# YannDubs/disentangling-vae

Hardware: NVIDIA H100
Metric: images/sec (higher is better)
Workload: dtype f32

## Files before the change

### disentangling-vae_b200/csrc/dv_conv_tc.cu

```cuda
#include "dv_common.cuh"
#include "dv_ptx.cuh"

namespace dv {
namespace tc {

using namespace ptx;

constexpr int kATile = 128 * 128;
constexpr int kBTap = 64 * 128;
constexpr int kBBytes = kTaps * kBTap;
constexpr int kConsumers = 8;
constexpr int kThreads = (kConsumers + 1) * 32;
constexpr int kSmemMax = 232448;

__device__ __forceinline__ void consumers_sync() { asm volatile("bar.sync 1, %0;" ::"n"(kConsumers * 32) : "memory"); }

__device__ __forceinline__ int b_lane_row(int lane) { return (lane >> 4) * 32 + (lane & 7); }
__device__ __forceinline__ int b_lane_col(int lane) { return (lane & 8) >> 1; }
__device__ __forceinline__ void load_b_tap(uint32_t tap_base, int nt, int ks, int b_row, int b_col, uint32_t (&bh)[2], uint32_t (&bl)[2]) {
  uint32_t r[4];
  ldsm_x4(tap_base + swz128(b_row + 8 * nt, 8 * ks + b_col), r);
  bh[0] = r[0]; bh[1] = r[1]; bl[0] = r[2]; bl[1] = r[3];
}

struct DownGeom {
  int B, H, W;
  int rows_per_tile;
  int num_tiles;
  long long total_px;
};
constexpr int kDownStages = 5;
struct DownBarriers {
  uint64_t raw_full[kDownStages], raw_empty[kDownStages];
  uint64_t b_full;
  float bias[32];
  float csum[kConsumers][32];
};
constexpr int kDownSmem = kBBytes + kDownStages * kATile + 1024 + 2048;
static_assert(sizeof(DownBarriers) <= 2048, "barrier block too large");
static_assert(kDownSmem <= kSmemMax, "smem");

__global__ void __launch_bounds__(kThreads, 1)
conv_down32_mma_kernel(const __grid_constant__ CUtensorMap tmap_a, const __grid_constant__ CUtensorMap tmap_b,
                       const float* __restrict__ bias, const float* __restrict__ mask, float* __restrict__ lo,
                       DownGeom g, int act, float* __restrict__ colsum_part,
                       const uint32_t* __restrict__ mask_bits, uint32_t* __restrict__ bits_out) {
  extern __shared__ uint8_t smem_raw[];
  uint8_t* smem = align1024(smem_raw);
  uint8_t* Bs = smem;
  uint8_t* Raw = smem + kBBytes;
  DownBarriers* bars = reinterpret_cast<DownBarriers*>(Raw + kDownStages * kATile);
  const int warp = threadIdx.x >> 5, lane = threadIdx.x & 31;
  if (threadIdx.x == 0) {
    for (int s = 0; s < kDownStages; ++s) { mbar_init(&bars->raw_full[s], 1); mbar_init(&bars->raw_empty[s], kConsumers); }
    mbar_init(&bars->b_full, 1);
    fence_mbar_init();
  }
  if (threadIdx.x < 32) bars->bias[threadIdx.x] = bias ? bias[threadIdx.x] : 0.f;
  __syncthreads();

  if (warp == kConsumers) {
    if (lane != 0) return;
    prefetch_tmap(&tmap_a); prefetch_tmap(&tmap_b);
    mbar_arrive_expect_tx(&bars->b_full, kBBytes);
    for (int tap = 0; tap < kTaps; ++tap) tma_load_2d(Bs + tap * kBTap, &tmap_b, &bars->b_full, 0, tap * 64);
    int stage = 0; uint32_t phase = 0;
    for (int tile = blockIdx.x; tile < g.num_tiles; tile += gridDim.x) {
      const int r0 = tile * g.rows_per_tile;
      const int b0 = r0 / g.H, i0 = r0 % g.H;
      if (tile + (int)gridDim.x < g.num_tiles) {
        const int rn = (tile + gridDim.x) * g.rows_per_tile;
        const int bn = rn / g.H, in_ = rn % g.H;
        for (int t4 = 0; t4 < 4; ++t4) tma_prefetch_4d(&tmap_a, 0, (t4 & 1), 2 * in_ + (t4 >> 1), bn);
      }
      for (int tap = 0; tap < kTaps; ++tap) {
        const int kh = tap >> 2, kw = tap & 3;
        mbar_wait(&bars->raw_empty[stage], phase ^ 1);
        mbar_arrive_expect_tx(&bars->raw_full[stage], kATile);
        tma_load_4d(Raw + stage * kATile, &tmap_a, &bars->raw_full[stage], 0, kw - 1, 2 * i0 - 1 + kh, b0);
        if (++stage == kDownStages) { stage = 0; phase ^= 1; }
      }
    }
    return;
  }

  const int gq = lane >> 2, t = lane & 3;
  const int b_row = b_lane_row(lane), b_col = b_lane_col(lane);
  const int r0 = warp * 16 + gq;
  const uint32_t bs = smem_u32(Bs), raw0 = smem_u32(Raw);
  float csum[4][2] = {};
  mbar_wait(&bars->b_full, 0);
  int stage = 0; uint32_t phase = 0;
  for (int tile = blockIdx.x; tile < g.num_tiles; tile += gridDim.x) {
    float tot[4][4] = {}, corr[4][4] = {};
    for (int tap = 0; tap < kTaps; ++tap) {
      mbar_wait(&bars->raw_full[stage], phase);
      const uint32_t a_base = raw0 + stage * kATile, b_base = bs + tap * kBTap;
      float mn[4][4] = {};
#pragma unroll
      for (int ks = 0; ks < 4; ++ks) {
        uint32_t a[4], ah[4], al[4];
        a[0] = lds32(a_base + swz128(r0, 8 * ks + t));
        a[1] = lds32(a_base + swz128(r0 + 8, 8 * ks + t));
        a[2] = lds32(a_base + swz128(r0, 8 * ks + t + 4));
        a[3] = lds32(a_base + swz128(r0 + 8, 8 * ks + t + 4));
#pragma unroll
        for (int e = 0; e < 4; ++e) split_tf32(a[e], ah[e], al[e]);
#pragma unroll
        for (int nt = 0; nt < 4; ++nt) {
          uint32_t bh[2], bl[2];
          load_b_tap(b_base, nt, ks, b_row, b_col, bh, bl);
          mma_3xtf32(mn[nt], corr[nt], ah, al, bh, bl);
        }
      }
      __syncwarp();
      if (lane == 0) mbar_arrive(&bars->raw_empty[stage]);
      if (++stage == kDownStages) { stage = 0; phase ^= 1; }
#pragma unroll
      for (int nt = 0; nt < 4; ++nt)
#pragma unroll
        for (int e = 0; e < 4; ++e) tot[nt][e] += mn[nt][e];
    }
#pragma unroll
    for (int h = 0; h < 2; ++h) {
      const long long p = (long long)tile * 128 + r0 + 8 * h;
      const bool valid = p < g.total_px;
      uint32_t mb = 0xffffffffu;
      if (mask_bits && valid) mb = __ldg(mask_bits + p);
      const float* mk = (mask && !mask_bits && valid) ? mask + p * 32 : nullptr;
      uint32_t ob = 0u;
#pragma unroll
      for (int nt = 0; nt < 4; ++nt) {
        const int c = nt * 8 + 2 * t;
        float v[2];
#pragma unroll
        for (int e = 0; e < 2; ++e) {
          float x = (tot[nt][2 * h + e] + corr[nt][2 * h + e]) + bars->bias[c + e];
          if (act == DV_ACT_RELU) x = fmaxf(x, 0.f);
          v[e] = ((mb >> (c + e)) & 1u) ? x : 0.f;
        }
        if (mk) {
          const float2 m2 = __ldg(reinterpret_cast<const float2*>(mk + c));
          v[0] = m2.x > 0.f ? v[0] : 0.f; v[1] = m2.y > 0.f ? v[1] : 0.f;
        }
        if (valid) *reinterpret_cast<float2*>(lo + p * 32 + c) = make_float2(v[0], v[1]);
        else v[0] = v[1] = 0.f;
        ob |= (v[0] > 0.f ? 1u : 0u) << c | (v[1] > 0.f ? 1u : 0u) << (c + 1);
        csum[nt][0] += v[0]; csum[nt][1] += v[1];
      }
      ob |= __shfl_xor_sync(0xffffffffu, ob, 1);
      ob |= __shfl_xor_sync(0xffffffffu, ob, 2);
      if (bits_out && valid && t == 0) bits_out[p] = ob;
    }
  }
  if (colsum_part) {
#pragma unroll
    for (int nt = 0; nt < 4; ++nt)
#pragma unroll
      for (int e = 0; e < 2; ++e) {
        float s = csum[nt][e];
        s += __shfl_xor_sync(0xffffffffu, s, 4);
        s += __shfl_xor_sync(0xffffffffu, s, 8);
        s += __shfl_xor_sync(0xffffffffu, s, 16);
        if (gq == 0) bars->csum[warp][nt * 8 + 2 * t + e] = s;
      }
    consumers_sync();
    if (warp == 0) {
      float s = 0.f;
      for (int w = 0; w < kConsumers; ++w) s += bars->csum[w][lane];
      colsum_part[blockIdx.x * 32 + lane] = s;
    }
  }
}

constexpr int kWtSlots = kConsumers;
struct WtBarriers {
  uint64_t raw_full[kWtSlots], raw_empty[kWtSlots];
  uint64_t l_full[2], l_empty[2];
  float lsum[kConsumers][32];
};
constexpr int kWtTotFloats = 2 * 32 * 32;
constexpr int kWtSmem = kWtSlots * kATile + 2 * kATile + 2048 + kConsumers * kWtTotFloats * 4 + 1024;
static_assert(sizeof(WtBarriers) <= 2048, "barrier block too large");
static_assert(kWtSmem <= kSmemMax, "smem");

struct WtGeom {
  int B, H, W, rows_per_tile, num_tiles, tiles_per_cta;
};

__global__ void __launch_bounds__(kThreads, 1)
conv_wgrad32_mma_kernel(const __grid_constant__ CUtensorMap tmap_hi, const __grid_constant__ CUtensorMap tmap_lo,
                        float* __restrict__ ws, WtGeom g) {
  extern __shared__ uint8_t smem_raw[];
  uint8_t* smem = align1024(smem_raw);
  uint8_t* Raw = smem;
  uint8_t* Ls = smem + kWtSlots * kATile;
  WtBarriers* bars = reinterpret_cast<WtBarriers*>(Ls + 2 * kATile);
  const int warp = threadIdx.x >> 5, lane = threadIdx.x & 31;
  float* tot = reinterpret_cast<float*>(Ls + 2 * kATile + 2048) + warp * kWtTotFloats + lane;
  const int t_begin = blockIdx.x * g.tiles_per_cta;
  const int t_end = min(g.num_tiles, t_begin + g.tiles_per_cta);

  if (threadIdx.x == 0) {
    for (int s = 0; s < kWtSlots; ++s) { mbar_init(&bars->raw_full[s], 1); mbar_init(&bars->raw_empty[s], 1); }
    for (int s = 0; s < 2; ++s) { mbar_init(&bars->l_full[s], 1); mbar_init(&bars->l_empty[s], kConsumers); }
    fence_mbar_init();
  }
  __syncthreads();

  if (warp == kConsumers) {
    if (lane != 0) return;
    prefetch_tmap(&tmap_hi); prefetch_tmap(&tmap_lo);
    uint32_t tseq = 0;
    for (int tile = t_begin; tile < t_end; ++tile, ++tseq) {
      const int r0 = tile * g.rows_per_tile;
      const int b0 = r0 / g.H, i0 = r0 % g.H;
      if (tile + 1 < t_end) {
        const int rn = (tile + 1) * g.rows_per_tile;
        const int bn = rn / g.H, in_ = rn % g.H;
        for (int t4 = 0; t4 < 4; ++t4) tma_prefetch_4d(&tmap_hi, 0, (t4 & 1), 2 * in_ + (t4 >> 1), bn);
        tma_prefetch_4d(&tmap_lo, 0, 0, in_, bn);
      }
      const int lb = tseq & 1;
      mbar_wait(&bars->l_empty[lb], ((tseq >> 1) & 1u) ^ 1u);
      mbar_arrive_expect_tx(&bars->l_full[lb], kATile);
      tma_load_4d(Ls + lb * kATile, &tmap_lo, &bars->l_full[lb], 0, 0, i0, b0);
      for (int tap = 0; tap < kTaps; ++tap) {
        const int kh = tap >> 2, kw = tap & 3, slot = tap & 7;
        const uint32_t use = tseq * 2 + (tap >> 3);
        mbar_wait(&bars->raw_empty[slot], (use & 1u) ^ 1u);
        mbar_arrive_expect_tx(&bars->raw_full[slot], kATile);
        tma_load_4d(Raw + slot * kATile, &tmap_hi, &bars->raw_full[slot], 0, kw - 1, 2 * i0 - 1 + kh, b0);
      }
    }
    return;
  }

  const int gq = lane >> 2, t = lane & 3;
  const uint32_t slot_base = smem_u32(Raw) + warp * kATile, l0 = smem_u32(Ls);
  for (int k = 0; k < 64; ++k) tot[k * 32] = 0.f;
  float lsum = 0.f;
  uint32_t tseq = 0;
  for (int tile = t_begin; tile < t_end; ++tile, ++tseq) {
    const int lb = tseq & 1;
    mbar_wait(&bars->l_full[lb], (tseq >> 1) & 1u);
    const uint32_t l_base = l0 + lb * kATile;
#pragma unroll 4
    for (int r = 0; r < 16; ++r) lsum += __uint_as_float(lds32(l_base + swz128(warp * 16 + r, lane)));
#pragma unroll 1
    for (int j = 0; j < 2; ++j) {
      const uint32_t use = tseq * 2 + j;
      mbar_wait(&bars->raw_full[warp], use & 1u);
      float mn[2][4][4] = {}, cr[2][4][4] = {};
#pragma unroll 1
      for (int ks = 0; ks < 16; ++ks) {
        const int px0 = 8 * ks + 2 * t, px1 = px0 + 1;
        uint32_t ah[2][4], al[2][4], bh[4][2], bl[4][2];
#pragma unroll
        for (int mt = 0; mt < 2; ++mt) {
          const int c = mt * 16 + gq;
          uint32_t a[4];
          a[0] = lds32(slot_base + swz128(px0, c));
          a[1] = lds32(slot_base + swz128(px0, c + 8));
          a[2] = lds32(slot_base + swz128(px1, c));
          a[3] = lds32(slot_base + swz128(px1, c + 8));
#pragma unroll
          for (int e = 0; e < 4; ++e) split_tf32(a[e], ah[mt][e], al[mt][e]);
        }
#pragma unroll
        for (int nt = 0; nt < 4; ++nt) {
          const int cl = nt * 8 + gq;
          split_tf32(lds32(l_base + swz128(px0, cl)), bh[nt][0], bl[nt][0]);
          split_tf32(lds32(l_base + swz128(px1, cl)), bh[nt][1], bl[nt][1]);
        }
#pragma unroll
        for (int mt = 0; mt < 2; ++mt)
#pragma unroll
          for (int nt = 0; nt < 4; ++nt) mma_3xtf32(mn[mt][nt], cr[mt][nt], ah[mt], al[mt], bh[nt], bl[nt]);
      }
      __syncwarp();
      if (lane == 0) mbar_arrive(&bars->raw_empty[warp]);
#pragma unroll
      for (int mt = 0; mt < 2; ++mt)
#pragma unroll
        for (int nt = 0; nt < 4; ++nt)
#pragma unroll
          for (int e = 0; e < 4; ++e) tot[(j * 32 + (mt * 4 + nt) * 4 + e) * 32] += mn[mt][nt][e] + cr[mt][nt][e];
    }
    __syncwarp();
    if (lane == 0) mbar_arrive(&bars->l_empty[lb]);
  }

  float* out = ws + (long long)blockIdx.x * (kTaps * 32 + 1) * kLoCh;
#pragma unroll
  for (int j = 0; j < 2; ++j) {
    const int tap = warp + 8 * j;
#pragma unroll
    for (int mt = 0; mt < 2; ++mt)
#pragma unroll
      for (int nt = 0; nt < 4; ++nt)
#pragma unroll
        for (int h = 0; h < 2; ++h) {
          const int c = mt * 16 + gq + 8 * h, cl = nt * 8 + 2 * t;
          *reinterpret_cast<float2*>(out + (tap * 32 + c) * kLoCh + cl) =
              make_float2(tot[(j * 32 + (mt * 4 + nt) * 4 + 2 * h) * 32], tot[(j * 32 + (mt * 4 + nt) * 4 + 2 * h + 1) * 32]);
        }
  }
  bars->lsum[warp][lane] = lsum;
  consumers_sync();
  if (warp == 0) {
    float s = 0.f;
    for (int w = 0; w < kConsumers; ++w) s += bars->lsum[w][lane];
    out[(kTaps * 32) * kLoCh + lane] = s;
  }
}

constexpr int kHaloStageBytes = 26 * 1024;
constexpr int kHaloStages = 3;
struct HaloGeom {
  int B, H, W, TR, TB, tiles_per_img, num_tiles, valid_rows, box_px, box_bytes;
};
struct HaloBarriers {
  uint64_t raw_full[kHaloStages], raw_empty[kHaloStages];
  uint64_t b_full;
  float bias[32];
};
constexpr int kHaloSmem = kBBytes + kHaloStages * kHaloStageBytes + 1024 + 1024;
static_assert(sizeof(HaloBarriers) <= 1024, "barrier block too large");
static_assert(kHaloSmem <= kSmemMax, "smem");

__global__ void __launch_bounds__(kThreads, 1)
conv_up_halo_mma_kernel(const __grid_constant__ CUtensorMap tmap_a, const __grid_constant__ CUtensorMap tmap_b,
                        const float* __restrict__ bias, const float* __restrict__ mask, float* __restrict__ hi_out,
                        HaloGeom g, int act, const uint32_t* __restrict__ mask_bits, uint32_t* __restrict__ bits_out) {
  extern __shared__ uint8_t smem_raw[];
  uint8_t* smem = align1024(smem_raw);
  uint8_t* Bs = smem;
  uint8_t* Raw = smem + kBBytes;
  HaloBarriers* bars = reinterpret_cast<HaloBarriers*>(Raw + kHaloStages * kHaloStageBytes);
  const int warp = threadIdx.x >> 5, lane = threadIdx.x & 31;

  if (threadIdx.x == 0) {
    for (int s = 0; s < kHaloStages; ++s) { mbar_init(&bars->raw_full[s], 1); mbar_init(&bars->raw_empty[s], kConsumers); }
    mbar_init(&bars->b_full, 1);
    fence_mbar_init();
  }
  if (threadIdx.x < 32) bars->bias[threadIdx.x] = bias ? bias[threadIdx.x] : 0.f;
  __syncthreads();

  if (warp == kConsumers) {
    if (lane != 0) return;
    prefetch_tmap(&tmap_a); prefetch_tmap(&tmap_b);
    mbar_arrive_expect_tx(&bars->b_full, kBBytes);
    for (int tap = 0; tap < kTaps; ++tap) tma_load_2d(Bs + tap * kBTap, &tmap_b, &bars->b_full, 0, tap * 64);
    uint32_t t_seq = 0;
    for (int tile = blockIdx.x; tile < g.num_tiles; tile += gridDim.x, ++t_seq) {
      const int stage = t_seq % kHaloStages;
      int b0, i0;
      if (g.TB > 1) { b0 = tile * g.TB; i0 = 0; } else { b0 = tile / g.tiles_per_img; i0 = (tile % g.tiles_per_img) * g.TR; }
      mbar_wait(&bars->raw_empty[stage], ((t_seq / kHaloStages) & 1u) ^ 1u);
      mbar_arrive_expect_tx(&bars->raw_full[stage], g.box_bytes);
      tma_load_4d(Raw + stage * kHaloStageBytes, &tmap_a, &bars->raw_full[stage], 0, 0, i0 - 1, b0);
    }
    return;
  }

  const int gq = lane >> 2, t = lane & 3;
  const int b_row = b_lane_row(lane), b_col = b_lane_col(lane);
  const int HH = 2 * g.H, WW = 2 * g.W;
  const uint32_t bs = smem_u32(Bs), raw0 = smem_u32(Raw);
  int rj[2], src0[2];
  bool row_ok[2];
#pragma unroll
  for (int h = 0; h < 2; ++h) {
    const int row = warp * 16 + gq + 8 * h;
    const int rt = row / g.W, rtb = rt / g.TR;
    rj[h] = row - rt * g.W;
    src0[h] = min((rtb * (g.TR + 2) + (rt - rtb * g.TR) + 1) * g.W + rj[h], g.box_px - 1);
    row_ok[h] = row < g.valid_rows;
  }
  mbar_wait(&bars->b_full, 0);
  uint32_t t_seq = 0;
  for (int tile = blockIdx.x; tile < g.num_tiles; tile += gridDim.x, ++t_seq) {
    const int stage = t_seq % kHaloStages;
    const uint32_t a_base = raw0 + stage * kHaloStageBytes;
    mbar_wait(&bars->raw_full[stage], (t_seq / kHaloStages) & 1u);
    int b0, i0;
    if (g.TB > 1) { b0 = tile * g.TB; i0 = 0; } else { b0 = tile / g.tiles_per_img; i0 = (tile % g.tiles_per_img) * g.TR; }
#pragma unroll 1
    for (int pidx = 0; pidx < 4; ++pidx) {
      const int ph = pidx >> 1, pw = pidx & 1;
      float tot[4][4] = {}, corr[4][4] = {};
#pragma unroll
      for (int s = 0; s < 9; ++s) {
        const int di = s / 3 - 1, dj = s % 3 - 1;
        const int kh = ph + 1 - 2 * di, kw = pw + 1 - 2 * dj;
        if (kh < 0 || kh > 3 || kw < 0 || kw > 3) continue;
        const uint32_t b_base = bs + (kh * 4 + kw) * kBTap;
        int p[2];
        uint32_t keep[2];
#pragma unroll
        for (int h = 0; h < 2; ++h) {
          const bool ok = row_ok[h] && (unsigned)(rj[h] + dj) < (unsigned)g.W;
          p[h] = ok ? src0[h] + di * g.W + dj : src0[h];
          keep[h] = ok ? 0xffffffffu : 0u;
        }
        float mn[4][4] = {};
#pragma unroll
        for (int ks = 0; ks < 4; ++ks) {
          uint32_t ah[4], al[4];
          split_tf32(lds32(a_base + swz128(p[0], 8 * ks + t)) & keep[0], ah[0], al[0]);
          split_tf32(lds32(a_base + swz128(p[1], 8 * ks + t)) & keep[1], ah[1], al[1]);
          split_tf32(lds32(a_base + swz128(p[0], 8 * ks + t + 4)) & keep[0], ah[2], al[2]);
          split_tf32(lds32(a_base + swz128(p[1], 8 * ks + t + 4)) & keep[1], ah[3], al[3]);
#pragma unroll
          for (int nt = 0; nt < 4; ++nt) {
            uint32_t bh[2], bl[2];
            load_b_tap(b_base, nt, ks, b_row, b_col, bh, bl);
            mma_3xtf32(mn[nt], corr[nt], ah, al, bh, bl);
          }
        }
#pragma unroll
        for (int nt = 0; nt < 4; ++nt)
#pragma unroll
          for (int e = 0; e < 4; ++e) tot[nt][e] += mn[nt][e];
      }
#pragma unroll
      for (int h = 0; h < 2; ++h) {
        const int r = warp * 16 + gq + 8 * h, tr = r / g.W;
        const int tb = tr / g.TR, rr = tr - tb * g.TR;
        const int b = b0 + tb, i = i0 + rr, j = r - tr * g.W;
        const bool valid = r < g.valid_rows && b < g.B && i < g.H;
        const long long opix = valid ? ((long long)(b * HH + 2 * i + ph) * WW + 2 * j + pw) : 0;
        uint32_t mb = 0xffffffffu;
        if (mask_bits && valid) mb = __ldg(mask_bits + opix);
        const float* mk = (mask && !mask_bits && valid) ? mask + opix * 32 : nullptr;
        uint32_t ob = 0u;
#pragma unroll
        for (int nt = 0; nt < 4; ++nt) {
          const int c = nt * 8 + 2 * t;
          float v[2];
#pragma unroll
          for (int e = 0; e < 2; ++e) {
            float x = (tot[nt][2 * h + e] + corr[nt][2 * h + e]) + bars->bias[c + e];
            if (act == DV_ACT_RELU) x = fmaxf(x, 0.f);
            v[e] = ((mb >> (c + e)) & 1u) ? x : 0.f;
          }
          if (mk) {
            const float2 m2 = __ldg(reinterpret_cast<const float2*>(mk + c));
            v[0] = m2.x > 0.f ? v[0] : 0.f; v[1] = m2.y > 0.f ? v[1] : 0.f;
          }
          if (valid) *reinterpret_cast<float2*>(hi_out + opix * 32 + c) = make_float2(v[0], v[1]);
          ob |= (v[0] > 0.f ? 1u : 0u) << c | (v[1] > 0.f ? 1u : 0u) << (c + 1);
        }
        ob |= __shfl_xor_sync(0xffffffffu, ob, 1);
        ob |= __shfl_xor_sync(0xffffffffu, ob, 2);
        if (bits_out && valid && t == 0) bits_out[opix] = ob;
      }
    }
    __syncwarp();
    if (lane == 0) mbar_arrive(&bars->raw_empty[stage]);
  }
}

constexpr int kPackMultiMax = 8;
struct ConvPackTable {
  const float* w[kPackMultiMax];
  float* wp[kPackMultiMax];
  int CH[kPackMultiMax];
};
__global__ void conv_pack_multi_kernel(ConvPackTable tab) {
  const float* __restrict__ w = tab.w[blockIdx.y];
  float* __restrict__ wp = tab.wp[blockIdx.y];
  const int CH = tab.CH[blockIdx.y];
  const int n = kLoCh * CH * kTaps;
  for (int idx = blockIdx.x * blockDim.x + threadIdx.x; idx < n; idx += gridDim.x * blockDim.x) {
    const int tap = idx % kTaps, c = (idx / kTaps) % CH, cl = idx / (kTaps * CH);
    const float v = w[idx];
    if (CH != 32) {
      wp[(tap * CH + c) * kLoCh + cl] = v;
      wp[n + (tap * CH + c) * kLoCh + cl] = v;
      continue;
    }
    float* wd = wp;
    float* wu = wp + kTaps * 64 * 32;
    const float hi = tf32_round(v);
    const float lo = tf32_round(v - hi);
    wd[(tap * 64 + cl) * 32 + c] = hi;
    wd[(tap * 64 + 32 + cl) * 32 + c] = lo;
    wu[(tap * 64 + c) * 32 + cl] = hi;
    wu[(tap * 64 + 32 + c) * 32 + cl] = lo;
  }
}

static bool make_act_tmap(CUtensorMap* m, const float* base, int B, int HH, int WW, int bw, int bh, int bb, int stride) {
  EncodeTiledFn enc = get_encode();
  if (!enc) return false;
  cuuint64_t gdim[4] = {32, (cuuint64_t)WW, (cuuint64_t)HH, (cuuint64_t)B};
  cuuint64_t gstr[3] = {128, (cuuint64_t)WW * 128, (cuuint64_t)HH * WW * 128};
  cuuint32_t box[4] = {32, (cuuint32_t)bw, (cuuint32_t)bh, (cuuint32_t)bb};
  cuuint32_t estr[4] = {1, (cuuint32_t)stride, (cuuint32_t)stride, 1};
  return enc(m, CU_TENSOR_MAP_DATA_TYPE_FLOAT32, 4, const_cast<float*>(base), gdim, gstr, box, estr,
             CU_TENSOR_MAP_INTERLEAVE_NONE, CU_TENSOR_MAP_SWIZZLE_128B, CU_TENSOR_MAP_L2_PROMOTION_L2_128B,
             CU_TENSOR_MAP_FLOAT_OOB_FILL_NONE) == CUDA_SUCCESS;
}
static bool make_w_tmap(CUtensorMap* m, const float* base) {
  EncodeTiledFn enc = get_encode();
  if (!enc) return false;
  cuuint64_t gdim[2] = {32, (cuuint64_t)kTaps * 64};
  cuuint64_t gstr[1] = {128};
  cuuint32_t box[2] = {32, 64};
  cuuint32_t estr[2] = {1, 1};
  return enc(m, CU_TENSOR_MAP_DATA_TYPE_FLOAT32, 2, const_cast<float*>(base), gdim, gstr, box, estr,
             CU_TENSOR_MAP_INTERLEAVE_NONE, CU_TENSOR_MAP_SWIZZLE_128B, CU_TENSOR_MAP_L2_PROMOTION_L2_128B,
             CU_TENSOR_MAP_FLOAT_OOB_FILL_NONE) == CUDA_SUCCESS;
}

int pack_multi(int n, const float* const* w, float* const* wp, const int* CH, cudaStream_t st) {
  for (int base = 0; base < n; base += kPackMultiMax) {
    ConvPackTable tab = {};
    const int m = n - base < kPackMultiMax ? n - base : kPackMultiMax;
    for (int i = 0; i < m; ++i) { tab.w[i] = w[base + i]; tab.wp[i] = wp[base + i]; tab.CH[i] = CH[base + i]; }
    conv_pack_multi_kernel<<<dim3(16, m), 256, 0, st>>>(tab);
    const int rc = check_launch();
    if (rc != DV_OK) return rc;
  }
  return DV_OK;
}

int conv_down32_tc(const float* hi, const float* wd_packed, const float* bias, const float* mask, float* lo,
                   int B, int H, int W, int act, cudaStream_t st, float* colsum_part, int* nparts,
                   const uint32_t* mask_bits, uint32_t* bits_out) {
  if (nparts) *nparts = 0;
  if (W > 128 || 128 % W != 0) return DV_ERR_BAD_SHAPE;
  DownGeom g = {};
  g.B = B; g.H = H; g.W = W;
  g.rows_per_tile = 128 / W;
  const int TR = g.rows_per_tile < H ? g.rows_per_tile : H;
  if (H % TR != 0 || g.rows_per_tile % TR != 0) return DV_ERR_BAD_SHAPE;
  const int TB = g.rows_per_tile / TR;
  g.total_px = (long long)B * H * W;
  g.num_tiles = (int)((g.total_px + 127) / 128);
  CUtensorMap ta, tb;
  if (!make_act_tmap(&ta, hi, B, 2 * H, 2 * W, 2 * W, 2 * TR, TB, 2)) return DV_ERR_CUDA;
  if (!make_w_tmap(&tb, wd_packed)) return DV_ERR_CUDA;
  static bool attr = false;
  const int rc = set_max_dynamic_smem(conv_down32_mma_kernel, kDownSmem, &attr);
  if (rc != DV_OK) return rc;
  const int grid = g.num_tiles < kNumSMs ? g.num_tiles : kNumSMs;
  conv_down32_mma_kernel<<<grid, kThreads, kDownSmem, st>>>(ta, tb, bias, mask, lo, g, act, colsum_part, mask_bits, bits_out);
  if (nparts && colsum_part) *nparts = grid;
  return check_launch();
}

int wgrad_splits(int B, int H, int W) {
  const int num_tiles = (int)(((long long)B * H * W + 127) / 128);
  const int grid = num_tiles < kNumSMs ? num_tiles : kNumSMs;
  const int tiles_per_cta = (num_tiles + grid - 1) / grid;
  return (num_tiles + tiles_per_cta - 1) / tiles_per_cta;
}

int conv_wgrad32_tc(const float* lo, const float* hi, float* ws, int B, int H, int W, cudaStream_t st) {
  if (W > 128 || 128 % W != 0) return DV_ERR_BAD_SHAPE;
  WtGeom g = {};
  g.B = B; g.H = H; g.W = W;
  g.rows_per_tile = 128 / W;
  const int TR = g.rows_per_tile < H ? g.rows_per_tile : H;
  if (H % TR != 0 || g.rows_per_tile % TR != 0) return DV_ERR_BAD_SHAPE;
  const int TB = g.rows_per_tile / TR;
  g.num_tiles = (int)(((long long)B * H * W + 127) / 128);
  const int grid = wgrad_splits(B, H, W);
  g.tiles_per_cta = (g.num_tiles + grid - 1) / grid;
  CUtensorMap thi, tlo;
  if (!make_act_tmap(&thi, hi, B, 2 * H, 2 * W, 2 * W, 2 * TR, TB, 2)) return DV_ERR_CUDA;
  if (!make_act_tmap(&tlo, lo, B, H, W, W, TR, TB, 1)) return DV_ERR_CUDA;
  static bool attr = false;
  const int rc = set_max_dynamic_smem(conv_wgrad32_mma_kernel, kWtSmem, &attr);
  if (rc != DV_OK) return rc;
  conv_wgrad32_mma_kernel<<<grid, kThreads, kWtSmem, st>>>(thi, tlo, ws, g);
  return check_launch();
}

int conv_up_halo(const float* lo, const float* wu, const float* bias, const float* mask, float* hi,
                 int B, int H, int W, int act, cudaStream_t st, const uint32_t* mask_bits, uint32_t* bits_out) {
  HaloGeom g = {};
  g.B = B; g.H = H; g.W = W;
  if (W > 32 || 128 % W != 0) return DV_ERR_BAD_SHAPE;
  const int rpt = 128 / W;
  if (rpt >= H) {
    g.TR = H;
    g.TB = rpt / H < 1 ? 1 : rpt / H;
    while (g.TB > 1 && g.TB * (H + 2) * W * 128 > kHaloStageBytes) --g.TB;
    g.tiles_per_img = 1;
    g.num_tiles = (B + g.TB - 1) / g.TB;
  } else {
    g.TR = rpt; g.TB = 1;
    g.tiles_per_img = (H + rpt - 1) / rpt;
    g.num_tiles = B * g.tiles_per_img;
  }
  g.valid_rows = g.TB * g.TR * W;
  g.box_px = g.TB * (g.TR + 2) * W;
  g.box_bytes = g.box_px * 128;
  if (g.box_bytes > kHaloStageBytes) return DV_ERR_BAD_SHAPE;
  CUtensorMap ta, tb;
  if (!make_act_tmap(&ta, lo, g.B, g.H, g.W, g.W, g.TR + 2, g.TB, 1)) return DV_ERR_CUDA;
  if (!make_w_tmap(&tb, wu)) return DV_ERR_CUDA;
  static bool attr = false;
  const int rc = set_max_dynamic_smem(conv_up_halo_mma_kernel, kHaloSmem, &attr);
  if (rc != DV_OK) return rc;
  const int grid = g.num_tiles < kNumSMs ? g.num_tiles : kNumSMs;
  conv_up_halo_mma_kernel<<<grid, kThreads, kHaloSmem, st>>>(ta, tb, bias, mask, hi, g, act, mask_bits, bits_out);
  return check_launch();
}

}
}
```

### disentangling-vae_b200/csrc/dv_ptx.cuh

```cuda
#pragma once
#include <cuda.h>
#include <cuda_runtime.h>
#include <stdint.h>

namespace dv {
namespace ptx {

__device__ __forceinline__ uint32_t smem_u32(const void* p) {
  return static_cast<uint32_t>(__cvta_generic_to_shared(p));
}

__device__ __forceinline__ void mbar_init(uint64_t* bar, uint32_t count) {
  asm volatile("mbarrier.init.shared::cta.b64 [%0], %1;" ::"r"(smem_u32(bar)), "r"(count));
}
__device__ __forceinline__ void fence_mbar_init() {
  asm volatile("fence.mbarrier_init.release.cluster;" ::: "memory");
}
__device__ __forceinline__ void mbar_arrive(uint64_t* bar) {
  asm volatile("mbarrier.arrive.shared::cta.b64 _, [%0];" ::"r"(smem_u32(bar)) : "memory");
}
__device__ __forceinline__ void mbar_arrive_expect_tx(uint64_t* bar, uint32_t bytes) {
  asm volatile("mbarrier.arrive.expect_tx.shared::cta.b64 _, [%0], %1;" ::"r"(smem_u32(bar)), "r"(bytes) : "memory");
}
__device__ __forceinline__ void mbar_wait(uint64_t* bar, uint32_t parity) {
  const uint32_t addr = smem_u32(bar);
  uint32_t done = 0;
  for (uint32_t spin = 0; !done; ++spin) {
    asm volatile(
        "{\n\t.reg .pred p;\n\t"
        "mbarrier.try_wait.parity.shared::cta.b64 p, [%1], %2;\n\t"
        "selp.u32 %0, 1, 0, p;\n\t}"
        : "=r"(done)
        : "r"(addr), "r"(parity)
        : "memory");
    if (spin > (1u << 24)) __trap();
  }
}

__device__ __forceinline__ uint32_t lds32(uint32_t smem_addr) {
  uint32_t v;
  asm volatile("ld.shared.u32 %0, [%1];" : "=r"(v) : "r"(smem_addr) : "memory");
  return v;
}

__device__ __forceinline__ void ldsm_x4(uint32_t smem_addr, uint32_t (&r)[4]) {
  asm volatile("ldmatrix.sync.aligned.m8n8.x4.shared.b16 {%0, %1, %2, %3}, [%4];"
               : "=r"(r[0]), "=r"(r[1]), "=r"(r[2]), "=r"(r[3])
               : "r"(smem_addr)
               : "memory");
}

__device__ __forceinline__ uint32_t swz128(int r, int c) {
  return (uint32_t)(r * 128 + ((((c >> 2) ^ (r & 7)) << 4) | ((c & 3) << 2)));
}

__device__ __forceinline__ void prefetch_tmap(const CUtensorMap* m) {
  asm volatile("prefetch.tensormap [%0];" ::"l"(reinterpret_cast<uint64_t>(m)) : "memory");
}
__device__ __forceinline__ void tma_load_4d(void* smem_dst, const CUtensorMap* m, uint64_t* bar, int c0, int c1, int c2, int c3) {
  asm volatile(
      "cp.async.bulk.tensor.4d.shared::cluster.global.mbarrier::complete_tx::bytes [%0], [%1, {%3, %4, %5, %6}], [%2];"
      ::"r"(smem_u32(smem_dst)), "l"(reinterpret_cast<uint64_t>(m)), "r"(smem_u32(bar)), "r"(c0), "r"(c1), "r"(c2), "r"(c3)
      : "memory");
}
__device__ __forceinline__ void tma_load_2d(void* smem_dst, const CUtensorMap* m, uint64_t* bar, int c0, int c1) {
  asm volatile(
      "cp.async.bulk.tensor.2d.shared::cluster.global.mbarrier::complete_tx::bytes [%0], [%1, {%3, %4}], [%2];"
      ::"r"(smem_u32(smem_dst)), "l"(reinterpret_cast<uint64_t>(m)), "r"(smem_u32(bar)), "r"(c0), "r"(c1)
      : "memory");
}
__device__ __forceinline__ void tma_prefetch_4d(const CUtensorMap* m, int c0, int c1, int c2, int c3) {
  asm volatile("cp.async.bulk.prefetch.tensor.4d.L2.global.tile [%0, {%1, %2, %3, %4}];"
               ::"l"(reinterpret_cast<uint64_t>(m)), "r"(c0), "r"(c1), "r"(c2), "r"(c3) : "memory");
}

typedef CUresult (*EncodeTiledFn)(CUtensorMap*, CUtensorMapDataType, cuuint32_t, void*, const cuuint64_t*, const cuuint64_t*,
                                  const cuuint32_t*, const cuuint32_t*, CUtensorMapInterleave, CUtensorMapSwizzle,
                                  CUtensorMapL2promotion, CUtensorMapFloatOOBfill);
inline EncodeTiledFn get_encode() {
  static const EncodeTiledFn fn = [] {
    void* p = nullptr;
    cudaDriverEntryPointQueryResult qres;
    const bool ok = cudaGetDriverEntryPoint("cuTensorMapEncodeTiled", &p, cudaEnableDefault, &qres) == cudaSuccess &&
                    qres == cudaDriverEntryPointSuccess;
    return ok ? reinterpret_cast<EncodeTiledFn>(p) : nullptr;
  }();
  return fn;
}

__device__ __forceinline__ float tf32_round(float x) {
  return __uint_as_float((__float_as_uint(x) + 0x1000u) & 0xFFFFE000u);
}
__device__ __forceinline__ void split_tf32(uint32_t x, uint32_t& hi, uint32_t& lo) {
  const float h = tf32_round(__uint_as_float(x));
  hi = __float_as_uint(h);
  lo = __float_as_uint(tf32_round(__uint_as_float(x) - h));
}

__device__ __forceinline__ void mma_tf32(float (&d)[4], const uint32_t (&a)[4], const uint32_t (&b)[2]) {
  asm volatile(
      "mma.sync.aligned.m16n8k8.row.col.f32.tf32.tf32.f32 {%0, %1, %2, %3}, {%4, %5, %6, %7}, {%8, %9}, {%0, %1, %2, %3};"
      : "+f"(d[0]), "+f"(d[1]), "+f"(d[2]), "+f"(d[3])
      : "r"(a[0]), "r"(a[1]), "r"(a[2]), "r"(a[3]), "r"(b[0]), "r"(b[1]));
}

__device__ __forceinline__ void mma_3xtf32(float (&main)[4], float (&corr)[4], const uint32_t (&a_hi)[4],
                                           const uint32_t (&a_lo)[4], const uint32_t (&b_hi)[2], const uint32_t (&b_lo)[2]) {
  mma_tf32(main, a_hi, b_hi);
  mma_tf32(corr, a_hi, b_lo);
  mma_tf32(corr, a_lo, b_hi);
}

}
}
```

Measured before the change: 427,000.

## Switch 3xTF32 conv MMAs from mma.sync to async wgmma with register A operand

Replaces the per-warp mma.sync m16n8k8 TF32 loops (with ldmatrix B loads) in the downsampling and transposed conv kernels with warpgroup wgmma m64n32k8 calls. A comes from registers and B is read straight from swizzled shared memory via descriptors. Accumulators are double-buffered across taps so one tap's wgmma can overlap the next tap's A loads and split, and the main accumulator is folded late. The transposed conv also replaces the 9-iteration loop with continue-skips by a direct 4-tap enumeration. The risks are that 8 consumer warps form two warpgroups whose descriptor and layout assumptions must match, and that register pressure rises from the 16-entry ah/al arrays and two accumulator sets.

```diff
diff --git a/disentangling-vae_b200/csrc/dv_conv_tc.cu b/disentangling-vae_b200/csrc/dv_conv_tc.cu
--- a/disentangling-vae_b200/csrc/dv_conv_tc.cu
+++ b/disentangling-vae_b200/csrc/dv_conv_tc.cu
@@ -15,12 +15,32 @@
 
 __device__ __forceinline__ void consumers_sync() { asm volatile("bar.sync 1, %0;" ::"n"(kConsumers * 32) : "memory"); }
 
-__device__ __forceinline__ int b_lane_row(int lane) { return (lane >> 4) * 32 + (lane & 7); }
-__device__ __forceinline__ int b_lane_col(int lane) { return (lane & 8) >> 1; }
-__device__ __forceinline__ void load_b_tap(uint32_t tap_base, int nt, int ks, int b_row, int b_col, uint32_t (&bh)[2], uint32_t (&bl)[2]) {
-  uint32_t r[4];
-  ldsm_x4(tap_base + swz128(b_row + 8 * nt, 8 * ks + b_col), r);
-  bh[0] = r[0]; bh[1] = r[1]; bl[0] = r[2]; bl[1] = r[3];
+__device__ __forceinline__ void fold_tap(float (&tot)[16], float (&acc)[16]) {
+  fence_regs(acc);
+#pragma unroll
+  for (int i = 0; i < 16; ++i) tot[i] += acc[i];
+}
+
+__device__ __forceinline__ void product(float (&acc)[16], float (&acc_prev)[16], float (&corr)[16], float (&tot)[16],
+                                        uint32_t (&ah)[16], uint32_t (&al)[16], uint32_t a_base, int p0, int p1,
+                                        uint32_t keep0, uint32_t keep1, int t, uint32_t tap_base, int corr_accumulate) {
+#pragma unroll
+  for (int ks = 0; ks < 4; ++ks) {
+    wgmma_wait<3>();
+    if (ks == 3) fold_tap(tot, acc_prev);
+    split_tf32(lds32(a_base + swz128(p0, 8 * ks + t)) & keep0, ah[4 * ks + 0], al[4 * ks + 0]);
+    split_tf32(lds32(a_base + swz128(p1, 8 * ks + t)) & keep1, ah[4 * ks + 1], al[4 * ks + 1]);
+    split_tf32(lds32(a_base + swz128(p0, 8 * ks + t + 4)) & keep0, ah[4 * ks + 2], al[4 * ks + 2]);
+    split_tf32(lds32(a_base + swz128(p1, 8 * ks + t + 4)) & keep1, ah[4 * ks + 3], al[4 * ks + 3]);
+    fence_regs(acc);
+    fence_regs(corr);
+    wgmma_fence();
+    const uint64_t w_hi = wgmma_desc_k128(tap_base + 32 * ks), w_lo = wgmma_desc_k128(tap_base + 32 * 128 + 32 * ks);
+    wgmma_m64n32k8_rs(acc, ah + 4 * ks, w_hi, ks);
+    wgmma_m64n32k8_rs(corr, ah + 4 * ks, w_lo, ks | corr_accumulate);
+    wgmma_m64n32k8_rs(corr, al + 4 * ks, w_hi, 1);
+    wgmma_commit();
+  }
 }
 
 struct DownGeom {
@@ -85,42 +105,31 @@
   }
 
   const int gq = lane >> 2, t = lane & 3;
-  const int b_row = b_lane_row(lane), b_col = b_lane_col(lane);
   const int r0 = warp * 16 + gq;
   const uint32_t bs = smem_u32(Bs), raw0 = smem_u32(Raw);
   float csum[4][2] = {};
   mbar_wait(&bars->b_full, 0);
   int stage = 0; uint32_t phase = 0;
+  uint32_t ah[16], al[16];
+  auto tap_product = [&](float (&acc)[16], float (&acc_prev)[16], float (&corr)[16], float (&tot)[16], int tap) {
+    mbar_wait(&bars->raw_full[stage], phase);
+    product(acc, acc_prev, corr, tot, ah, al, raw0 + stage * kATile, r0, r0 + 8, ~0u, ~0u, t, bs + tap * kBTap, tap);
+    __syncwarp();
+    if (lane == 0) mbar_arrive(&bars->raw_empty[stage]);
+    if (++stage == kDownStages) { stage = 0; phase ^= 1; }
+  };
   for (int tile = blockIdx.x; tile < g.num_tiles; tile += gridDim.x) {
-    float tot[4][4] = {}, corr[4][4] = {};
-    for (int tap = 0; tap < kTaps; ++tap) {
-      mbar_wait(&bars->raw_full[stage], phase);
-      const uint32_t a_base = raw0 + stage * kATile, b_base = bs + tap * kBTap;
-      float mn[4][4] = {};
-#pragma unroll
-      for (int ks = 0; ks < 4; ++ks) {
-        uint32_t a[4], ah[4], al[4];
-        a[0] = lds32(a_base + swz128(r0, 8 * ks + t));
-        a[1] = lds32(a_base + swz128(r0 + 8, 8 * ks + t));
-        a[2] = lds32(a_base + swz128(r0, 8 * ks + t + 4));
-        a[3] = lds32(a_base + swz128(r0 + 8, 8 * ks + t + 4));
-#pragma unroll
-        for (int e = 0; e < 4; ++e) split_tf32(a[e], ah[e], al[e]);
-#pragma unroll
-        for (int nt = 0; nt < 4; ++nt) {
-          uint32_t bh[2], bl[2];
-          load_b_tap(b_base, nt, ks, b_row, b_col, bh, bl);
-          mma_3xtf32(mn[nt], corr[nt], ah, al, bh, bl);
-        }
-      }
-      __syncwarp();
-      if (lane == 0) mbar_arrive(&bars->raw_empty[stage]);
-      if (++stage == kDownStages) { stage = 0; phase ^= 1; }
-#pragma unroll
-      for (int nt = 0; nt < 4; ++nt)
-#pragma unroll
-        for (int e = 0; e < 4; ++e) tot[nt][e] += mn[nt][e];
-    }
+    float tot[16] = {}, corr[16], acc[2][16];
+#pragma unroll
+    for (int i = 0; i < 16; ++i) acc[1][i] = 0.f;
+#pragma unroll 1
+    for (int tap = 0; tap < kTaps; tap += 2) {
+      tap_product(acc[0], acc[1], corr, tot, tap);
+      tap_product(acc[1], acc[0], corr, tot, tap + 1);
+    }
+    wgmma_wait<0>();
+    fold_tap(tot, acc[1]);
+    fence_regs(corr);
 #pragma unroll
     for (int h = 0; h < 2; ++h) {
       const long long p = (long long)tile * 128 + r0 + 8 * h;
@@ -135,7 +144,7 @@
         float v[2];
 #pragma unroll
         for (int e = 0; e < 2; ++e) {
-          float x = (tot[nt][2 * h + e] + corr[nt][2 * h + e]) + bars->bias[c + e];
+          float x = (tot[4 * nt + 2 * h + e] + corr[4 * nt + 2 * h + e]) + bars->bias[c + e];
           if (act == DV_ACT_RELU) x = fmaxf(x, 0.f);
           v[e] = ((mb >> (c + e)) & 1u) ? x : 0.f;
         }
@@ -366,7 +375,6 @@
   }
 
   const int gq = lane >> 2, t = lane & 3;
-  const int b_row = b_lane_row(lane), b_col = b_lane_col(lane);
   const int HH = 2 * g.H, WW = 2 * g.W;
   const uint32_t bs = smem_u32(Bs), raw0 = smem_u32(Raw);
   int rj[2], src0[2];
@@ -379,6 +387,7 @@
     src0[h] = min((rtb * (g.TR + 2) + (rt - rtb * g.TR) + 1) * g.W + rj[h], g.box_px - 1);
     row_ok[h] = row < g.valid_rows;
   }
+  uint32_t ah[16], al[16];
   mbar_wait(&bars->b_full, 0);
   uint32_t t_seq = 0;
   for (int tile = blockIdx.x; tile < g.num_tiles; tile += gridDim.x, ++t_seq) {
@@ -390,13 +399,13 @@
 #pragma unroll 1
     for (int pidx = 0; pidx < 4; ++pidx) {
       const int ph = pidx >> 1, pw = pidx & 1;
-      float tot[4][4] = {}, corr[4][4] = {};
-#pragma unroll
-      for (int s = 0; s < 9; ++s) {
-        const int di = s / 3 - 1, dj = s % 3 - 1;
-        const int kh = ph + 1 - 2 * di, kw = pw + 1 - 2 * dj;
-        if (kh < 0 || kh > 3 || kw < 0 || kw > 3) continue;
-        const uint32_t b_base = bs + (kh * 4 + kw) * kBTap;
+      float tot[16] = {}, corr[16], acc[2][16];
+#pragma unroll
+      for (int i = 0; i < 16; ++i) acc[1][i] = 0.f;
+#pragma unroll
+      for (int q = 0; q < 4; ++q) {
+        const int di = ph - 1 + (q >> 1), dj = pw - 1 + (q & 1);
+        const uint32_t b_base = bs + ((3 - ph - 2 * (q >> 1)) * 4 + 3 - pw - 2 * (q & 1)) * kBTap;
         int p[2];
         uint32_t keep[2];
 #pragma unroll
@@ -405,26 +414,11 @@
           p[h] = ok ? src0[h] + di * g.W + dj : src0[h];
           keep[h] = ok ? 0xffffffffu : 0u;
         }
-        float mn[4][4] = {};
-#pragma unroll
-        for (int ks = 0; ks < 4; ++ks) {
-          uint32_t ah[4], al[4];
-          split_tf32(lds32(a_base + swz128(p[0], 8 * ks + t)) & keep[0], ah[0], al[0]);
-          split_tf32(lds32(a_base + swz128(p[1], 8 * ks + t)) & keep[1], ah[1], al[1]);
-          split_tf32(lds32(a_base + swz128(p[0], 8 * ks + t + 4)) & keep[0], ah[2], al[2]);
-          split_tf32(lds32(a_base + swz128(p[1], 8 * ks + t + 4)) & keep[1], ah[3], al[3]);
-#pragma unroll
-          for (int nt = 0; nt < 4; ++nt) {
-            uint32_t bh[2], bl[2];
-            load_b_tap(b_base, nt, ks, b_row, b_col, bh, bl);
-            mma_3xtf32(mn[nt], corr[nt], ah, al, bh, bl);
-          }
-        }
-#pragma unroll
-        for (int nt = 0; nt < 4; ++nt)
-#pragma unroll
-          for (int e = 0; e < 4; ++e) tot[nt][e] += mn[nt][e];
-      }
+        product(acc[q & 1], acc[(q + 1) & 1], corr, tot, ah, al, a_base, p[0], p[1], keep[0], keep[1], t, b_base, q);
+      }
+      wgmma_wait<0>();
+      fold_tap(tot, acc[1]);
+      fence_regs(corr);
 #pragma unroll
       for (int h = 0; h < 2; ++h) {
         const int r = warp * 16 + gq + 8 * h, tr = r / g.W;
@@ -442,7 +436,7 @@
           float v[2];
 #pragma unroll
           for (int e = 0; e < 2; ++e) {
-            float x = (tot[nt][2 * h + e] + corr[nt][2 * h + e]) + bars->bias[c + e];
+            float x = (tot[4 * nt + 2 * h + e] + corr[4 * nt + 2 * h + e]) + bars->bias[c + e];
             if (act == DV_ACT_RELU) x = fmaxf(x, 0.f);
             v[e] = ((mb >> (c + e)) & 1u) ? x : 0.f;
           }
diff --git a/disentangling-vae_b200/csrc/dv_ptx.cuh b/disentangling-vae_b200/csrc/dv_ptx.cuh
--- a/disentangling-vae_b200/csrc/dv_ptx.cuh
+++ b/disentangling-vae_b200/csrc/dv_ptx.cuh
@@ -41,13 +41,6 @@
   uint32_t v;
   asm volatile("ld.shared.u32 %0, [%1];" : "=r"(v) : "r"(smem_addr) : "memory");
   return v;
-}
-
-__device__ __forceinline__ void ldsm_x4(uint32_t smem_addr, uint32_t (&r)[4]) {
-  asm volatile("ldmatrix.sync.aligned.m8n8.x4.shared.b16 {%0, %1, %2, %3}, [%4];"
-               : "=r"(r[0]), "=r"(r[1]), "=r"(r[2]), "=r"(r[3])
-               : "r"(smem_addr)
-               : "memory");
 }
 
 __device__ __forceinline__ uint32_t swz128(int r, int c) {
@@ -111,5 +104,29 @@
   mma_tf32(corr, a_lo, b_hi);
 }
 
+__device__ __forceinline__ uint64_t wgmma_desc_k128(uint32_t smem_addr) {
+  return (uint64_t)((smem_addr & 0x3FFFFu) >> 4) | ((uint64_t)1 << 16) | ((uint64_t)(1024 >> 4) << 32) | ((uint64_t)1 << 62);
+}
+__device__ __forceinline__ void wgmma_fence() { asm volatile("wgmma.fence.sync.aligned;" ::: "memory"); }
+__device__ __forceinline__ void wgmma_commit() { asm volatile("wgmma.commit_group.sync.aligned;" ::: "memory"); }
+template <int N>
+__device__ __forceinline__ void wgmma_wait() { asm volatile("wgmma.wait_group.sync.aligned %0;" ::"n"(N) : "memory"); }
+template <int N>
+__device__ __forceinline__ void fence_regs(float (&r)[N]) {
+#pragma unroll
+  for (int i = 0; i < N; ++i) asm volatile("" : "+f"(r[i])::"memory");
+}
+
+__device__ __forceinline__ void wgmma_m64n32k8_rs(float (&d)[16], const uint32_t* a, uint64_t b_desc, int accumulate) {
+  asm volatile(
+      "{\n\t.reg .pred p;\n\tsetp.ne.b32 p, %21, 0;\n\t"
+      "wgmma.mma_async.sync.aligned.m64n32k8.f32.tf32.tf32 "
+      "{%0, %1, %2, %3, %4, %5, %6, %7, %8, %9, %10, %11, %12, %13, %14, %15}, "
+      "{%16, %17, %18, %19}, %20, p, 1, 1;\n\t}"
+      : "+f"(d[0]), "+f"(d[1]), "+f"(d[2]), "+f"(d[3]), "+f"(d[4]), "+f"(d[5]), "+f"(d[6]), "+f"(d[7]),
+        "+f"(d[8]), "+f"(d[9]), "+f"(d[10]), "+f"(d[11]), "+f"(d[12]), "+f"(d[13]), "+f"(d[14]), "+f"(d[15])
+      : "r"(a[0]), "r"(a[1]), "r"(a[2]), "r"(a[3]), "l"(b_desc), "r"(accumulate));
+}
+
 }
 }
```

Measured after the change: 447,700 (median of 6 runs). 4.9% higher.
